# spotify-research/llark

Hardware: AMD Instinct MI355X
Metric: clips/sec (25 s audio + 128-tok prompt) end-to-end fwd (higher is better)
Workload: dtype fp16x2-split(fp32-class) prior + bf16x2-split(fp32-class) llm; 1 GPU; configs[1]+llm: 8x25s clips -> Jukebox VQ-VAE+36-layer prior -> 240x4800 -> projector -> Llama-2-7B fwd (S=371) logits; clips_per_gpu=8, global_batch=8, audio_samples=1048576, seq_len=371, prior_depth=36, prior_precision=f16x2, prior_layernorm_folded=True, parallelism=dp1 (clip-sharded, no collective), debug_overrides=False

## Files before the change

llark_amd/csrc/llama.hip:

```cpp
#include <stdlib.h>

#include "common.h"

namespace llark {

template <typename T>
__global__ void embed_gather_kernel(const long long* __restrict__ ids, const T* __restrict__ table,
                                    float* __restrict__ out, int rows, int width, int vocab, int ldo) {
    const int row = blockIdx.x;
    long long id = ids[row];
    id = id < 0 ? 0 : (id >= vocab ? vocab - 1 : id);
    const T* src = table + (size_t)id * width;
    float* dst = out + (size_t)row * ldo;
    for (int c = threadIdx.x; c < width; c += blockDim.x) dst[c] = (float)src[c];
}

template <int NV>
__global__ __launch_bounds__(256) void rmsnorm_kernel(const float* __restrict__ x, int ldx, int rows, int width,
                                                      const float* __restrict__ w, float eps,
                                                      bf16_t* __restrict__ hi, bf16_t* __restrict__ lo, int ldo) {
    const int lane = threadIdx.x & 63;
    const int row = blockIdx.x * 4 + (threadIdx.x >> 6);
    if (row >= rows) return;
    const int w4 = width >> 2;
    const float4* xr = (const float4*)(x + (size_t)row * ldx);
    const float4* w4p = (const float4*)w;
    float4 v[NV], gw[NV];
#pragma unroll
    for (int k = 0; k < NV; ++k) {
        const int c = lane + 64 * k;
        if (c < w4) {
            v[k] = xr[c];
            gw[k] = w4p[c];
        } else {
            v[k] = gw[k] = make_float4(0.f, 0.f, 0.f, 0.f);
        }
    }
    float s = 0.0f;
#pragma unroll
    for (int k = 0; k < NV; ++k)
        if (lane + 64 * k < w4) s += (v[k].x * v[k].x + v[k].y * v[k].y) + (v[k].z * v[k].z + v[k].w * v[k].w);
    const float var = wave_sum(s) / (float)width;
    const float rstd = 1.0f / sqrtf(var + eps);
    bf16x4_t* hr = (bf16x4_t*)(hi + (size_t)row * ldo);
    bf16x4_t* lr = lo ? (bf16x4_t*)(lo + (size_t)row * ldo) : nullptr;
#pragma unroll
    for (int k = 0; k < NV; ++k) {
        const int c = lane + 64 * k;
        if (c < w4) {
            const float4 g = gw[k];
            float y[4] = {g.x * (v[k].x * rstd), g.y * (v[k].y * rstd), g.z * (v[k].z * rstd), g.w * (v[k].w * rstd)};
            bf16x4_t h, l;
#pragma unroll
            for (int e = 0; e < 4; ++e) {
                h[e] = (bf16_t)y[e];
                l[e] = (bf16_t)(y[e] - (float)h[e]);
            }
            hr[c] = h;
            if (lr) lr[c] = l;
        }
    }
}

__device__ __forceinline__ void store_split(bf16_t* __restrict__ hi, bf16_t* __restrict__ lo, size_t idx, float v) {
    const bf16_t h = (bf16_t)v;
    hi[idx] = h;
    if (lo) lo[idx] = (bf16_t)(v - (float)h);
}

__global__ __launch_bounds__(256) void rope_split_kernel(const float* __restrict__ qkv, int S, int nh, int pos0,
                                                         const float* __restrict__ cos_t, const float* __restrict__ sin_t,
                                                         bf16_t* __restrict__ q, bf16_t* __restrict__ kc,
                                                         bf16_t* __restrict__ vtc, bf16_t* __restrict__ q_lo,
                                                         bf16_t* __restrict__ kc_lo, bf16_t* __restrict__ vtc_lo, int smax,
                                                         const int* __restrict__ pos_dev) {
    __shared__ float sv[64][129];
    if (pos_dev) pos0 = *pos_dev;
    const int hd = 128, H = nh * hd;
    const int s0 = blockIdx.x * 64, h = blockIdx.y, b = blockIdx.z;
    const int ns = (S - s0) < 64 ? (S - s0) : 64;
    for (int i = threadIdx.x; i < ns * 64; i += 256) {
        const int t = i >> 6, d = i & 63;
        const int s = s0 + t, pos = pos0 + s;
        const float* row = qkv + ((size_t)b * S + s) * 3 * H + h * hd;
        const float c = cos_t[(size_t)pos * 64 + d], sn = sin_t[(size_t)pos * 64 + d];
        const float q1 = row[d], q2 = row[d + 64], k1 = row[H + d], k2 = row[H + d + 64];
        const float qa = __fadd_rn(__fmul_rn(q1, c), __fmul_rn(-q2, sn));
        const float qb = __fadd_rn(__fmul_rn(q2, c), __fmul_rn(q1, sn));
        const float ka = __fadd_rn(__fmul_rn(k1, c), __fmul_rn(-k2, sn));
        const float kb = __fadd_rn(__fmul_rn(k2, c), __fmul_rn(k1, sn));
        const size_t qo = (((size_t)b * nh + h) * S + s) * hd;
        const size_t ko = (((size_t)b * nh + h) * smax + pos) * hd;
        store_split(q, q_lo, qo + d, qa);
        store_split(q, q_lo, qo + d + 64, qb);
        store_split(kc, kc_lo, ko + d, ka);
        store_split(kc, kc_lo, ko + d + 64, kb);
    }
    for (int i = threadIdx.x; i < ns * hd; i += 256) {
        const int t = i >> 7, d = i & 127;
        sv[t][d] = qkv[((size_t)b * S + s0 + t) * 3 * H + 2 * H + h * hd + d];
    }
    __syncthreads();
    for (int i = threadIdx.x; i < hd * 64; i += 256) {
        const int d = i >> 6, t = i & 63;
        if (t < ns) store_split(vtc, vtc_lo, (((size_t)b * nh + h) * hd + d) * smax + pos0 + s0 + t, sv[t][d]);
    }
}

__device__ __forceinline__ int k_swz(int key) { return ((key & 3) << 1) | (key & 8); }
__device__ __forceinline__ int k_off(int key, int chunk) { return key * 256 + ((chunk ^ k_swz(key)) << 4); }
__device__ __forceinline__ int v_off(int d, int chunk) { return d * 128 + ((chunk ^ ((d >> 1) & 7)) << 4); }
__device__ __forceinline__ int sub_row(int sub, int i) { return ((sub >> 1) << 5) + ((i >> 2) << 3) + ((sub & 1) << 2) + (i & 3); }

#ifndef ATTN_PREFILL_SM2
#define ATTN_PREFILL_SM2 1
#endif
#ifndef ATTN_PREFILL_PF
#define ATTN_PREFILL_PF 3
#endif
template <bool SPLIT, int NQ, bool P2, bool ALIBI, bool VARLEN = false>
__global__ __launch_bounds__(256) __attribute__((amdgpu_waves_per_eu((NQ == 1 && !SPLIT) ? 3 : 2, (NQ == 1 && !SPLIT) ? 3 : 2))) void attn_prefill_kernel(const bf16_t* __restrict__ q, const bf16_t* __restrict__ kc,
                                                           const bf16_t* __restrict__ vtc, const bf16_t* __restrict__ q_lo,
                                                           const bf16_t* __restrict__ kc_lo, const bf16_t* __restrict__ vtc_lo,
                                                           bf16_t* __restrict__ out, bf16_t* __restrict__ out_lo,
                                                           int S_arg, int nh, int nbh, int past, int smax, float scale,
                                                           const float* __restrict__ alibi_arg, float* __restrict__ lse, int paired,
                                                           const AttnSeqs<VARLEN> vl) {
    extern __shared__ __attribute__((aligned(16))) char smem[];
    const float* alibi = ALIBI ? alibi_arg : nullptr;
    char* sKl = smem + 32768;
    char* sVl = smem + 49152;
    constexpr int BQ = 64 * NQ;
    constexpr float LOG2E = 1.4426950408889634f;
    const int lane = threadIdx.x & 63;
    const int wv = __builtin_amdgcn_readfirstlane(threadIdx.x >> 6);
    const int g = lane >> 4, c = lane & 15;
    const int nt_grid = (S_arg + BQ - 1) / BQ;
    const int np = paired ? (nt_grid + 1) >> 1 : nt_grid;
    int pidx, bhid;
    {
        const int L = blockIdx.x;
        if ((nbh & 7) == 0) {
            bhid = (L & 7) + 8 * (L / (8 * np));
            pidx = (L >> 3) % np;
        } else {
            bhid = L / np;
            pidx = L - bhid * np;
        }
    }
    const int b = bhid / nh, h = bhid - b * nh;
    int S = S_arg, nt = nt_grid;
    size_t qrow0 = (size_t)bhid * S_arg;
    size_t krow0 = (size_t)bhid * smax;
    size_t vcol0 = (size_t)bhid * 128 * smax;
    size_t orow0 = (size_t)b * S_arg;
    if constexpr (VARLEN) {
        int off, len;
        if (!attn_seq_of(vl, b, S_arg, off, len)) return;
        S = len;
        nt = (S + BQ - 1) / BQ;
        if (pidx >= (paired ? (nt + 1) >> 1 : nt)) return;
        qrow0 = (size_t)h * vl.s_total + off;
        krow0 = (size_t)h * smax + off;
        vcol0 = (size_t)h * 128 * smax + off;
        orow0 = (size_t)off;
    }
    const int total = past + S;
    const float slope2 = alibi ? alibi[h] * LOG2E : 0.0f;
    const float scale2 = scale * LOG2E;
    const bf16_t* qb = q + qrow0 * 128;
    const bf16_t* kb = kc + krow0 * 128;
    const bf16_t* vb = vtc + vcol0;
    const bf16_t* kbl = SPLIT ? kc_lo + krow0 * 128 : nullptr;
    const bf16_t* vbl = SPLIT ? vtc_lo + vcol0 : nullptr;

    constexpr int NST = SPLIT ? 1 : 2;
    constexpr int STAGE_BYTES = 32768;
    auto stage_regs = [&](const bf16_t* kbase, const bf16_t* vbase, char* dK, char* dV, int key0) __attribute__((always_inline)) {
        int tid_ = threadIdx.x;
        if constexpr (!SPLIT) asm volatile("" : "+v"(tid_));
#pragma unroll
        for (int i = 0; i < 4; ++i) {
            const int idx = tid_ + i * 256;
            {
                const int key = idx >> 4, ch = idx & 15;
                uint4 val = make_uint4(0, 0, 0, 0);
                if (key0 + key < total) val = *(const uint4*)(kbase + (size_t)(key0 + key) * 128 + ch * 8);
                *(uint4*)(dK + k_off(key, ch)) = val;
            }
            {
                const int d = idx >> 3, ch = idx & 7;
                uint4 val = make_uint4(0, 0, 0, 0);
                const int kk = key0 + ch * 8;
                if (kk + 7 < total) {
                    val = *(const uint4*)(vbase + (size_t)d * smax + kk);
                } else if (kk < total) {
                    const bf16_t* src = vbase + (size_t)d * smax + kk;
                    unsigned short tmp[8];
#pragma unroll
                    for (int e = 0; e < 8; ++e) tmp[e] = (kk + e < total) ? ((const unsigned short*)src)[e] : (unsigned short)0;
                    val = *(uint4*)tmp;
                }
                *(uint4*)(dV + v_off(d, ch)) = val;
            }
        }
    };
    unsigned dko[4], dvo[4];
#pragma unroll
    for (int i = 0; i < 4; ++i) {
        const int j = wv * 4 + i;
        const int krow = 4 * j + (lane >> 4);
        dko[i] = (unsigned)(krow * 128 + (((lane & 15) ^ k_swz(krow)) << 3)) * 2u;
        const int d = 8 * j + (lane >> 3);
        dvo[i] = (unsigned)(d * smax + (((lane & 7) ^ ((d >> 1) & 7)) << 3)) * 2u;
    }
    auto stage_dma = [&](char* dK, char* dV, int key0) __attribute__((always_inline)) {
        const char* kt_base = (const char*)(kb + (size_t)key0 * 128);
        const char* vt_base = (const char*)(vb + key0);
#pragma unroll
        for (int i = 0; i < 4; ++i) {
            const int j = wv * 4 + i;
            __builtin_amdgcn_global_load_lds((const __attribute__((address_space(1))) void*)(kt_base + dko[i]),
                                             (__attribute__((address_space(3))) void*)(dK + j * 1024), 16, 0, 0);
            __builtin_amdgcn_global_load_lds((const __attribute__((address_space(1))) void*)(vt_base + dvo[i]),
                                             (__attribute__((address_space(3))) void*)(dV + j * 1024), 16, 0, 0);
        }
    };
    auto stage = [&](int kt) __attribute__((always_inline)) {
        const int key0 = kt * 64;
        char* base = smem + (NST == 2 ? (kt & 1) * STAGE_BYTES : 0);
        if (!SPLIT && key0 + 64 <= total) {
            stage_dma(base, base + 16384, key0);
        } else {
            stage_regs(kb, vb, base, base + 16384, key0);
            if (SPLIT) {
                __builtin_amdgcn_sched_barrier(0);
                stage_regs(kbl, vbl, sKl, sVl, key0);
            }
        }
    };
    int kaddr[4], vaddr[2];
    {
        const int krow0 = 8 * (c >> 2) + (c & 3);
#pragma unroll
        for (int ks = 0; ks < 4; ++ks) kaddr[ks] = k_off(krow0, ks * 4 + g);
#pragma unroll
        for (int p = 0; p < 2; ++p) vaddr[p] = v_off(c, p * 4 + g);
    }
    auto ksub = [](int sub) { return (32 * (sub >> 1) + 4 * (sub & 1)) * 256; };
#pragma nounroll
    for (int pass = 0; pass < 2; ++pass) {
        const int tile = pass == 0 ? nt - 1 - pidx : pidx;
        if (pass == 1 && (!paired || tile == nt - 1 - pidx)) break;
        if (pass == 1) __syncthreads();
        const int q0 = tile * BQ;
        const int wq0 = q0 + wv * 16 * NQ;
        bf16x8_t qf[NQ][4], ql[SPLIT ? NQ : 1][4];
#pragma unroll
        for (int u = 0; u < NQ; ++u) {
            int qr = wq0 + u * 16 + c;
            qr = qr < S ? qr : S - 1;
#pragma unroll
            for (int ks = 0; ks < 4; ++ks) {
                qf[u][ks] = *(const bf16x8_t*)(qb + (size_t)qr * 128 + ks * 32 + g * 8);
                if (SPLIT) ql[u][ks] = *(const bf16x8_t*)(q_lo + qrow0 * 128 + (size_t)qr * 128 + ks * 32 + g * 8);
            }
        }
        f32x4_t o[NQ][8];
        float m_run[NQ], l_run[NQ];
#pragma unroll
        for (int u = 0; u < NQ; ++u) {
#pragma unroll
            for (int dt = 0; dt < 8; ++dt) o[u][dt] = f32x4_t{0.f, 0.f, 0.f, 0.f};
            m_run[u] = -INFINITY;
            l_run[u] = 0.0f;
        }

        int last_key = past + q0 + BQ - 1;
        if (last_key > total - 1) last_key = total - 1;
        const int ntiles = last_key / 64 + 1;

        if (NST == 2) stage(0);
        for (int kt = 0; kt < ntiles; ++kt) {
            const int key0 = kt * 64;
            if (NST == 2) {
                asm volatile("s_waitcnt vmcnt(0)" ::: "memory");
                __syncthreads();
                if (kt + 1 < ntiles) stage(kt + 1);
            } else {
                __syncthreads();
                stage(kt);
                __syncthreads();
            }
            const char* sK = smem + (NST == 2 ? (kt & 1) * STAGE_BYTES : 0);
            const char* sV = sK + 16384;
            if (key0 > past + wq0 + 16 * NQ - 1) continue;
            f32x4_t st[NQ][4];
            constexpr bool PF = !SPLIT && !ALIBI && (ATTN_PREFILL_PF & 1), PFV = !SPLIT && !ALIBI && NQ == 2 && (ATTN_PREFILL_PF & 2);
            bf16x8_t vfa[PFV ? 8 : 1];
            if constexpr (PF) {
                bf16x8_t kfa[2][4];
#pragma unroll
                for (int sub = 0; sub < 4; ++sub) {
                    kfa[0][sub] = *(const bf16x8_t*)(sK + kaddr[0] + ksub(sub));
#pragma unroll
                    for (int u = 0; u < NQ; ++u) st[u][sub] = f32x4_t{0.f, 0.f, 0.f, 0.f};
                }
#pragma unroll
                for (int ks = 0; ks < 4; ++ks) {
                    __builtin_amdgcn_sched_barrier(0);
                    if (ks < 3) {
#pragma unroll
                        for (int sub = 0; sub < 4; ++sub) kfa[(ks + 1) & 1][sub] = *(const bf16x8_t*)(sK + kaddr[ks + 1] + ksub(sub));
                    }
                    __builtin_amdgcn_sched_barrier(0);
#pragma unroll
                    for (int sub = 0; sub < 4; ++sub)
#pragma unroll
                        for (int u = 0; u < NQ; ++u) st[u][sub] = __builtin_amdgcn_mfma_f32_16x16x32_bf16(kfa[ks & 1][sub], qf[u][ks], st[u][sub], 0, 0, 0);
                }
            } else {
#pragma unroll
            for (int sub = 0; sub < 4; ++sub) {
#pragma unroll
                for (int u = 0; u < NQ; ++u) st[u][sub] = f32x4_t{0.f, 0.f, 0.f, 0.f};
#pragma unroll
                for (int ks = 0; ks < 4; ++ks) {
                    const bf16x8_t kf = *(const bf16x8_t*)(sK + kaddr[ks] + ksub(sub));
                    bf16x8_t kfl;
                    if (SPLIT) kfl = *(const bf16x8_t*)(sKl + kaddr[ks] + ksub(sub));
#pragma unroll
                    for (int u = 0; u < NQ; ++u) {
                        st[u][sub] = __builtin_amdgcn_mfma_f32_16x16x32_bf16(kf, qf[u][ks], st[u][sub], 0, 0, 0);
                        if (SPLIT) {
                            st[u][sub] = __builtin_amdgcn_mfma_f32_16x16x32_bf16(kfl, qf[u][ks], st[u][sub], 0, 0, 0);
                            st[u][sub] = __builtin_amdgcn_mfma_f32_16x16x32_bf16(kf, ql[u][ks], st[u][sub], 0, 0, 0);
                        }
                    }
                }
            }
            }
            if constexpr (PFV) {
                __builtin_amdgcn_sched_barrier(0);
#pragma unroll
                for (int dt = 0; dt < 8; ++dt) vfa[dt] = *(const bf16x8_t*)(sV + vaddr[0] + dt * 2048);
                __builtin_amdgcn_sched_barrier(0);
            }
            const bool need_mask = key0 + 63 > past + wq0 || key0 + 63 >= total;
            bf16x8_t ph[NQ][2], pl[P2 ? NQ : 1][2];
            constexpr bool SM2 = !SPLIT && !P2 && !ALIBI && ATTN_PREFILL_SM2;
            if constexpr (SM2) {
#pragma unroll
                for (int u = 0; u < NQ; ++u) {
                    const int lim = past + wq0 + u * 16 + c;
                    if (need_mask) {
#pragma unroll
                        for (int sub = 0; sub < 4; ++sub)
#pragma unroll
                            for (int r = 0; r < 4; ++r) {
                                const int key = key0 + sub_row(sub, 4 * g + r);
                                if (key > lim || key >= total) st[u][sub][r] = -INFINITY;
                            }
                    }
                    float mloc = fmaxf(fmaxf(st[u][0][0], st[u][0][1]), fmaxf(st[u][0][2], st[u][0][3]));
#pragma unroll
                    for (int sub = 1; sub < 4; ++sub) mloc = fmaxf(fmaxf(fmaxf(st[u][sub][0], st[u][sub][1]), fmaxf(st[u][sub][2], st[u][sub][3])), mloc);
                    {
                        const unsigned xm = __builtin_bit_cast(unsigned, mloc);
                        const auto a = __builtin_amdgcn_permlane16_swap(xm, xm, false, false);
                        const unsigned a0 = a[0], a1 = a[1];
                        mloc = fmaxf(__builtin_bit_cast(float, a0), __builtin_bit_cast(float, a1));
                        const unsigned ym = __builtin_bit_cast(unsigned, mloc);
                        const auto b2 = __builtin_amdgcn_permlane32_swap(ym, ym, false, false);
                        const unsigned b0 = b2[0], b1 = b2[1];
                        mloc = fmaxf(__builtin_bit_cast(float, b0), __builtin_bit_cast(float, b1));
                    }
                    const float mn = fmaxf(m_run[u], mloc * scale2);
                    const bool dead = mn == -INFINITY;
                    const float alpha = dead ? 1.0f : __builtin_amdgcn_exp2f(m_run[u] - mn);
                    const float nmn = dead ? 0.0f : -mn;
                    float rs = 0.0f;
#pragma unroll
                    for (int sub = 0; sub < 4; ++sub)
#pragma unroll
                        for (int r = 0; r < 4; ++r) {
                            const float pv = __builtin_amdgcn_exp2f(__builtin_fmaf(st[u][sub][r], scale2, nmn));
                            rs += pv;
                            ph[u][sub >> 1][(sub & 1) * 4 + r] = (bf16_t)pv;
                        }
                l_run[u] = l_run[u] * alpha + rs;
                    m_run[u] = mn;
                    if (__builtin_amdgcn_ballot_w64(alpha != 1.0f) != 0) {
#pragma unroll
                        for (int dt = 0; dt < 8; ++dt)
#pragma unroll
                            for (int r = 0; r < 4; ++r) o[u][dt][r] *= alpha;
                    }
                }
            } else
#pragma unroll
            for (int u = 0; u < NQ; ++u) {
                const int lim = past + wq0 + u * 16 + c;
                float mloc = -INFINITY;
                if (need_mask || alibi) {
#pragma unroll
                    for (int sub = 0; sub < 4; ++sub)
#pragma unroll
                        for (int r = 0; r < 4; ++r) {
                            const int key = key0 + sub_row(sub, 4 * g + r);
                            float sv = st[u][sub][r] * scale2;
                            if (alibi) sv += slope2 * (float)(key - (total - 1));
                            if (key > lim || key >= total) sv = -INFINITY;
                            st[u][sub][r] = sv;
                            mloc = fmaxf(mloc, sv);
                        }
                } else {
#pragma unroll
                    for (int sub = 0; sub < 4; ++sub)
#pragma unroll
                        for (int r = 0; r < 4; ++r) {
                            st[u][sub][r] *= scale2;
                            mloc = fmaxf(mloc, st[u][sub][r]);
                        }
                }
                mloc = fmaxf(mloc, __shfl_xor(mloc, 16, 64));
                mloc = fmaxf(mloc, __shfl_xor(mloc, 32, 64));
                const float mn = fmaxf(m_run[u], mloc);
                const bool dead = mn == -INFINITY;
                const float alpha = dead ? 1.0f : __builtin_amdgcn_exp2f(m_run[u] - mn);
                float rs = 0.0f;
#pragma unroll
                for (int sub = 0; sub < 4; ++sub)
#pragma unroll
                    for (int r = 0; r < 4; ++r) {
                        const float pv = dead ? 0.0f : __builtin_amdgcn_exp2f(st[u][sub][r] - mn);
                        rs += pv;
                        const bf16_t pb = (bf16_t)pv;
                        ph[u][sub >> 1][(sub & 1) * 4 + r] = pb;
                        if (P2) pl[u][sub >> 1][(sub & 1) * 4 + r] = (bf16_t)(pv - (float)pb);
                    }
                rs += __shfl_xor(rs, 16, 64);
                rs += __shfl_xor(rs, 32, 64);
                l_run[u] = l_run[u] * alpha + rs;
                m_run[u] = mn;
                if (__builtin_amdgcn_ballot_w64(alpha != 1.0f) != 0) {
#pragma unroll
                    for (int dt = 0; dt < 8; ++dt)
#pragma unroll
                        for (int r = 0; r < 4; ++r) o[u][dt][r] *= alpha;
                }
            }
            bf16x8_t vfb[PFV ? 8 : 1];
            if constexpr (PFV) {
                __builtin_amdgcn_sched_barrier(0);
#pragma unroll
                for (int dt = 0; dt < 8; ++dt) vfb[dt] = *(const bf16x8_t*)(sV + vaddr[1] + dt * 2048);
            }
#pragma unroll
            for (int p = 0; p < 2; ++p) {
#pragma unroll
                for (int dt = 0; dt < 8; ++dt) {
                    bf16x8_t vf;
                    if constexpr (PFV) vf = p == 0 ? vfa[dt] : vfb[dt];
                    else vf = *(const bf16x8_t*)(sV + vaddr[p] + dt * 2048);
                    bf16x8_t vfl;
                    if (SPLIT) vfl = *(const bf16x8_t*)(sVl + vaddr[p] + dt * 2048);
#pragma unroll
                    for (int u = 0; u < NQ; ++u) {
                        o[u][dt] = __builtin_amdgcn_mfma_f32_16x16x32_bf16(vf, ph[u][p], o[u][dt], 0, 0, 0);
                        if (P2) o[u][dt] = __builtin_amdgcn_mfma_f32_16x16x32_bf16(vf, pl[u][p], o[u][dt], 0, 0, 0);
                        if (SPLIT) o[u][dt] = __builtin_amdgcn_mfma_f32_16x16x32_bf16(vfl, ph[u][p], o[u][dt], 0, 0, 0);
                    }
                }
            }
        }
#pragma unroll
        for (int u = 0; u < NQ; ++u) {
            const int qi = wq0 + u * 16 + c;
            if (!SPLIT && !P2 && !ALIBI && ATTN_PREFILL_SM2) {
                l_run[u] += __shfl_xor(l_run[u], 16, 64);
                l_run[u] += __shfl_xor(l_run[u], 32, 64);
            }
            if (qi >= S) continue;
            const float inv = l_run[u] > 0.0f ? 1.0f / l_run[u] : 0.0f;
            if (lse && g == 0) lse[qrow0 + qi] = (m_run[u] + log2f(l_run[u])) * 0.6931471805599453f;
            const size_t dst = (orow0 + qi) * (size_t)(nh * 128) + h * 128;
#pragma unroll
            for (int dt = 0; dt < 8; ++dt) {
                bf16x4_t hi4, lo4;
#pragma unroll
                for (int r = 0; r < 4; ++r) {
                    const float v = o[u][dt][r] * inv;
                    hi4[r] = (bf16_t)v;
                    lo4[r] = (bf16_t)(v - (float)hi4[r]);
                }
                *(bf16x4_t*)(out + dst + dt * 16 + 4 * g) = hi4;
                if (SPLIT) *(bf16x4_t*)(out_lo + dst + dt * 16 + 4 * g) = lo4;
            }
        }
    }
}

template <bool SPLIT, bool P2>
static void launch_attn_prefill(hipStream_t st, const bf16_t* q, const bf16_t* kc, const bf16_t* vtc, const bf16_t* q_lo,
                                const bf16_t* kc_lo, const bf16_t* vtc_lo, bf16_t* out, bf16_t* out_lo, int batch, int s, int nh,
                                int past, int smax, float scale, const float* alibi, float* lse) {
    const int lds = 65536;
    const int nbh = batch * nh;
    auto pairs_ok = [&](int nt) { const long wgs = (long)((nt + 1) / 2) * nbh; return nt >= 2 && (wgs >= 2048 || wgs == 512 || wgs == 1024); };
    auto go = [&](auto alibi_c) {
        constexpr bool AL = decltype(alibi_c)::value;
        auto run = [&](auto nq_c) {
            constexpr int NQ = decltype(nq_c)::value;
            const int nt = cdiv(s, 64 * NQ), pr = pairs_ok(nt);
            static PerDeviceOnce once;
            if (once.first()) (void)hipFuncSetAttribute((const void*)attn_prefill_kernel<SPLIT, NQ, P2, AL>, hipFuncAttributeMaxDynamicSharedMemorySize, lds);
            attn_prefill_kernel<SPLIT, NQ, P2, AL><<<(pr ? (nt + 1) / 2 : nt) * nbh, 256, lds, st>>>(q, kc, vtc, q_lo, kc_lo, vtc_lo, out, out_lo, s, nh, nbh, past,
                                                                                           smax, scale, alibi, lse, pr, AttnSeqs<false>{});
        };
        if (!SPLIT && (long)cdiv(s, 128) * nbh >= 1024) run(std::integral_constant<int, SPLIT ? 1 : 2>{});
        else run(std::integral_constant<int, 1>{});
    };
    if (alibi) go(std::true_type{});
    else go(std::false_type{});
}

template <int NW, int UBT>
__device__ __forceinline__ void attn_decode_body(const float* sq, float* sp, float* red, const bf16_t* kc, const bf16_t* vtc,
                                                 const bf16_t* kc_lo, const bf16_t* vtc_lo, bf16_t* __restrict__ out,
                                                 bf16_t* __restrict__ out_lo, int nh, int total, int smax, float scale,
                                                 const float* __restrict__ alibi) {
    constexpr int NT = NW * 64;
    constexpr int UB = UBT;
    constexpr int PARTS = NT / 128;
    const int h = blockIdx.x, b = blockIdx.y;
    const size_t bh = (size_t)b * nh + h;
    const int tid = threadIdx.x, lane = tid & 63, wv = tid >> 6;
    __syncthreads();
    const bf16_t* kb = kc + bh * (size_t)smax * 128;
    const bf16_t* kbl = kc_lo ? kc_lo + bh * (size_t)smax * 128 : nullptr;
    const int chunk = lane & 15, sub = lane >> 4;
    float qv[8];
#pragma unroll
    for (int e = 0; e < 8; ++e) qv[e] = sq[chunk * 8 + e];
    float lmax = -INFINITY;
    constexpr int KSTEP = NW * 4;
    for (int jb = wv * 4 + sub; jb < total + KSTEP - 1; jb += KSTEP * UB) {
        bf16x8_t kv[UB], kl[UB];
#pragma unroll
        for (int u = 0; u < UB; ++u) {
            int j = jb + KSTEP * u;
            j = j < total ? j : total - 1;
            kv[u] = *(const bf16x8_t*)(kb + (size_t)j * 128 + chunk * 8);
            if (kbl) kl[u] = *(const bf16x8_t*)(kbl + (size_t)j * 128 + chunk * 8);
        }
#pragma unroll
        for (int u = 0; u < UB; ++u) {
            const int j = jb + KSTEP * u;
            float s = 0.0f;
            if (kbl) {
#pragma unroll
                for (int e = 0; e < 8; ++e) s = fmaf(qv[e], (float)kv[u][e] + (float)kl[u][e], s);
            } else {
#pragma unroll
                for (int e = 0; e < 8; ++e) s = fmaf(qv[e], (float)kv[u][e], s);
            }
            s += __shfl_xor(s, 1, 64);
            s += __shfl_xor(s, 2, 64);
            s += __shfl_xor(s, 4, 64);
            s += __shfl_xor(s, 8, 64);
            s *= scale;
            if (alibi) s += alibi[blockIdx.x] * (float)(j - (total - 1));
            if (j < total) {
                if (chunk == 0) sp[j] = s;
                lmax = fmaxf(lmax, s);
            }
        }
    }
    lmax = wave_max(lmax);
    if (lane == 0) red[wv] = lmax;
    __syncthreads();
    float mx = red[0];
#pragma unroll
    for (int i = 1; i < NW; ++i) mx = fmaxf(mx, red[i]);
    float lsum = 0.0f;
    const int tpad = (total + 7) & ~7;
    for (int j = tid; j < tpad; j += NT) {
        float p = 0.0f;
        if (j < total) {
            p = expf(sp[j] - mx);
            lsum += p;
        }
        sp[j] = p;
    }
    lsum = wave_sum(lsum);
    __syncthreads();
    if (lane == 0) red[NW + wv] = lsum;
    __syncthreads();
    float tot = 0.0f;
#pragma unroll
    for (int i = 0; i < NW; ++i) tot += red[NW + i];
    const float inv = 1.0f / tot;
    const int d = tid / PARTS, part = tid % PARTS;
    const bf16_t* vr = vtc + (bh * 128 + d) * (size_t)smax;
    const bf16_t* vrl = vtc_lo ? vtc_lo + (bh * 128 + d) * (size_t)smax : nullptr;
    float acc = 0.0f;
    for (int cb = part * 8; cb < tpad; cb += 8 * PARTS * UB) {
        bf16x8_t vv[UB], vl[UB];
#pragma unroll
        for (int u = 0; u < UB; ++u) {
            int c8 = cb + 8 * PARTS * u;
            c8 = c8 < tpad ? c8 : tpad - 8;
            vv[u] = *(const bf16x8_t*)(vr + c8);
            if (vrl) vl[u] = *(const bf16x8_t*)(vrl + c8);
        }
#pragma unroll
        for (int u = 0; u < UB; ++u) {
            const int c8 = cb + 8 * PARTS * u;
            if (c8 < tpad) {
                if (vrl && c8 + 8 > total) {
#pragma unroll
                    for (int e = 0; e < 8; ++e)
                        if (c8 + e < total) acc = fmaf(sp[c8 + e], (float)vv[u][e] + (float)vl[u][e], acc);
                } else if (vrl) {
#pragma unroll
                    for (int e = 0; e < 8; ++e) acc = fmaf(sp[c8 + e], (float)vv[u][e] + (float)vl[u][e], acc);
                } else {
#pragma unroll
                    for (int e = 0; e < 8; ++e) acc = fmaf(sp[c8 + e], (float)vv[u][e], acc);
                }
            }
        }
    }
#pragma unroll
    for (int o = 1; o < PARTS; o <<= 1) acc += __shfl_xor(acc, o, 64);
    if (part == 0) store_split(out, out_lo, (size_t)b * (nh * 128) + h * 128 + d, acc * inv);
}

template <int NW, int UBT, bool ROWS = false>
__global__ __launch_bounds__(NW * 64, (NW >= 16 && UBT == 4) ? 7 : 1) void attn_decode_kernel(const bf16_t* __restrict__ q, bf16_t* kc, bf16_t* vtc,
                                                              const bf16_t* __restrict__ q_lo, bf16_t* kc_lo, bf16_t* vtc_lo,
                                                              bf16_t* __restrict__ out, bf16_t* __restrict__ out_lo,
                                                              int nh, int total, int smax, float scale,
                                                              const int* __restrict__ pos_dev, const float* __restrict__ alibi,
                                                              const float* __restrict__ qkv, const float* __restrict__ cos_t,
                                                              const float* __restrict__ sin_t, unsigned* chain_done) {
    extern __shared__ __attribute__((aligned(16))) char smem[];
    if constexpr (ROWS) {
        const int p = pos_dev[blockIdx.y];
        if (p < 0 || p >= smax) {
            if (threadIdx.x < 128)
                store_split(out, out_lo, (size_t)blockIdx.y * (nh * 128) + blockIdx.x * 128 + threadIdx.x, 0.0f);
            return;
        }
        total = p + 1;
    } else if (pos_dev) total = *pos_dev + 1;
    float* sp = (float*)smem;
    __shared__ float sq[128];
    __shared__ float red[2 * NW];
    const int h = blockIdx.x, b = blockIdx.y;
    const size_t bh = (size_t)b * nh + h;
    const int tid = threadIdx.x, lane = tid & 63, wv = tid >> 6;
    if (qkv) {
        const int pos = total - 1, H = nh * 128;
        const float* row = qkv + (size_t)b * 3 * H + h * 128;
        const bool split = kc_lo != nullptr;
        if (tid < 64) {
            const int d = tid;
            const float c = cos_t[(size_t)pos * 64 + d], sn = sin_t[(size_t)pos * 64 + d];
            const float q1 = row[d], q2 = row[d + 64], k1 = row[H + d], k2 = row[H + d + 64];
            const float qa = __fadd_rn(__fmul_rn(q1, c), __fmul_rn(-q2, sn));
            const float qb = __fadd_rn(__fmul_rn(q2, c), __fmul_rn(q1, sn));
            const float ka = __fadd_rn(__fmul_rn(k1, c), __fmul_rn(-k2, sn));
            const float kb2 = __fadd_rn(__fmul_rn(k2, c), __fmul_rn(k1, sn));
            const bf16_t ha = (bf16_t)qa, hb = (bf16_t)qb;
            sq[d] = (float)ha + (split ? (float)(bf16_t)(qa - (float)ha) : 0.0f);
            sq[d + 64] = (float)hb + (split ? (float)(bf16_t)(qb - (float)hb) : 0.0f);
            const size_t ko = (bh * (size_t)smax + pos) * 128;
            store_split(kc, kc_lo, ko + d, ka);
            store_split(kc, kc_lo, ko + d + 64, kb2);
        } else if (tid >= 128 && tid < 256) {
            const int d = tid - 128;
            store_split(vtc, vtc_lo, (bh * 128 + d) * (size_t)smax + pos, row[2 * H + d]);
        }
    } else if (tid < 128) {
        sq[tid] = (float)q[bh * 128 + tid] + (q_lo ? (float)q_lo[bh * 128 + tid] : 0.0f);
    }
    attn_decode_body<NW, UBT>(sq, sp, red, kc, vtc, kc_lo, vtc_lo, out, out_lo, nh, total, smax, scale, alibi);
    chain_signal(ChainSync{nullptr, 0u, chain_done});
}

__device__ __forceinline__ float clamp_keep_nan(float v, float lim) {
    return (lim > 0.0f && v == v) ? fminf(fmaxf(v, -lim), lim) : v;
}

template <int NW, int UBT>
__global__ __launch_bounds__(NW * 64, (NW >= 16 && UBT == 4) ? 7 : 1) void mpt_attn_decode_kernel(
    const float* __restrict__ qkv, int ldq, int nh, const int* __restrict__ pos_rows, float clip, const float* __restrict__ q_ln_w,
    const float* __restrict__ q_ln_b, const float* __restrict__ k_ln_w, const float* __restrict__ k_ln_b, float eps, bf16_t* kc, bf16_t* vtc,
    bf16_t* kc_lo, bf16_t* vtc_lo, int smax, bf16_t* __restrict__ out, bf16_t* __restrict__ out_lo, float scale,
    const float* __restrict__ alibi) {
    extern __shared__ __attribute__((aligned(16))) char smem[];
    const int pos = pos_rows[blockIdx.y];
    if (pos < 0 || pos >= smax) {
        if (threadIdx.x < 128) store_split(out, out_lo, (size_t)blockIdx.y * (nh * 128) + blockIdx.x * 128 + threadIdx.x, 0.0f);
        return;
    }
    float* sp = (float*)smem;
    __shared__ float sq[128];
    __shared__ float red[2 * NW];
    __shared__ float stat[4];
    const int h = blockIdx.x, b = blockIdx.y, H = nh * 128;
    const size_t bh = (size_t)b * nh + h;
    const int tid = threadIdx.x, lane = tid & 63, wv = tid >> 6;
    const float* row = qkv + (size_t)b * ldq;
    const bool ln = q_ln_w != nullptr, split = kc_lo != nullptr;
    const int d = tid & 127, isk = tid >> 7;
    float x = 0.0f, g = 1.0f, be = 0.0f;
    if (tid < 256) {
        x = clamp_keep_nan(row[isk * H + h * 128 + d], clip);
        if (ln) {
            g = (isk ? k_ln_w : q_ln_w)[h * 128 + d];
            const float* bp = isk ? k_ln_b : q_ln_b;
            be = bp ? bp[h * 128 + d] : 0.0f;
        }
    }
    if (tid >= 128 && tid < 256)
        store_split(vtc, vtc_lo, (bh * 128 + d) * (size_t)smax + pos, clamp_keep_nan(row[2 * H + h * 128 + d], clip));
    if (ln) {
        if (wv < 2) {
            const float4* xr = (const float4*)(row + wv * H);
            const int w4 = H >> 2;
            float s = 0.0f;
            for (int c = lane; c < w4; c += 64) {
                float4 v = xr[c];
                v.x = clamp_keep_nan(v.x, clip), v.y = clamp_keep_nan(v.y, clip), v.z = clamp_keep_nan(v.z, clip), v.w = clamp_keep_nan(v.w, clip);
                s += (v.x + v.y) + (v.z + v.w);
            }
            const float mean = wave_sum(s) / (float)H;
            float q = 0.0f;
            for (int c = lane; c < w4; c += 64) {
                float4 v = xr[c];
                v.x = clamp_keep_nan(v.x, clip), v.y = clamp_keep_nan(v.y, clip), v.z = clamp_keep_nan(v.z, clip), v.w = clamp_keep_nan(v.w, clip);
                const float a = v.x - mean, bb = v.y - mean, cc = v.z - mean, dd = v.w - mean;
                q += (a * a + bb * bb) + (cc * cc + dd * dd);
            }
            const float rstd = 1.0f / sqrtf(wave_sum(q) / (float)H + eps);
            if (lane == 0) stat[2 * wv] = mean, stat[2 * wv + 1] = rstd;
        }
        __syncthreads();
        if (tid < 256) x = (x - stat[2 * isk]) * stat[2 * isk + 1] * g + be;
    }
    if (tid < 128) {
        const bf16_t hi = (bf16_t)x;
        sq[d] = (float)hi + (split ? (float)(bf16_t)(x - (float)hi) : 0.0f);
    } else if (tid < 256) {
        store_split(kc, kc_lo, (bh * (size_t)smax + pos) * 128 + d, x);
    }
    attn_decode_body<NW, UBT>(sq, sp, red, kc, vtc, kc_lo, vtc_lo, out, out_lo, nh, pos + 1, smax, scale, alibi);
}

enum AttnDecodePos { POS_HOST, POS_DEV, POS_ROWS };
struct AttnDecodeArgs {
    const char* name;
    bool fused;
    const void *q, *q_lo;
    const float *qkv, *cos_t, *sin_t, *alibi;
    void *k_cache, *vt_cache, *k_cache_lo, *vt_cache_lo, *out, *out_lo;
    int batch, nh, hd, smax, max_pos;
    AttnDecodePos from;
    long total;
    const int *pos_dev, *pos_rows;
    unsigned* chain_done;
    llark_stream_t stream;
};

static int attn_decode(const AttnDecodeArgs& a) {
    LLARK_REQUIRE(a.k_cache && a.vt_cache && a.out && (a.fused ? a.qkv && a.cos_t && a.sin_t : a.q != nullptr) &&
                      (a.from == POS_HOST || (a.from == POS_DEV ? a.pos_dev : a.pos_rows)), "%s: null pointer", a.name);
    LLARK_REQUIRE(a.hd == 128, "%s: head_dim must be 128 (Llama-2), got %d", a.name, a.hd);
    LLARK_REQUIRE(!a.fused || ((a.k_cache_lo == nullptr) == (a.vt_cache_lo == nullptr) && (a.k_cache_lo == nullptr) == (a.out_lo == nullptr)),
                  "%s: give all lo planes (fp32-class mode) or none", a.name);
    bool ok = a.batch > 0 && a.nh > 0 && a.smax % 8 == 0;
    if (a.from == POS_HOST) ok = ok && a.total > 0 && a.total <= a.smax && (!a.fused || a.total <= a.max_pos);
    if (a.from == POS_DEV) ok = ok && (a.fused || a.smax > 0);
    if (a.from == POS_ROWS) ok = ok && a.smax > 0 && a.smax <= a.max_pos;
    LLARK_REQUIRE(ok, "%s: bad shape batch=%d nh=%d pos=%ld smax=%d max_pos=%d", a.name, a.batch, a.nh, a.total - 1, a.smax, a.max_pos);
    const size_t lds = (a.from == POS_HOST ? (size_t)((a.total + 7) & ~7L) : (size_t)a.smax) * sizeof(float);
    LLARK_REQUIRE(lds <= 128 * 1024, "%s: context too long for the LDS score buffer (total=%ld smax=%d)", a.name, a.total, a.smax);
    const float scale = (float)(1.0 / sqrt((double)a.hd));
    const int total = a.from == POS_HOST ? (int)a.total : 1;
    auto go = [&](auto rows_c) {
        constexpr bool ROWS = decltype(rows_c)::value;
        auto launch = [&](auto kern, int threads) {
            kern<<<dim3(a.nh, a.batch), threads, lds, (hipStream_t)a.stream>>>(
                (const bf16_t*)a.q, (bf16_t*)a.k_cache, (bf16_t*)a.vt_cache, (const bf16_t*)a.q_lo, (bf16_t*)a.k_cache_lo, (bf16_t*)a.vt_cache_lo,
                (bf16_t*)a.out, (bf16_t*)a.out_lo, a.nh, total, a.smax, scale, ROWS ? a.pos_rows : a.pos_dev, a.alibi, a.qkv, a.cos_t, a.sin_t, a.chain_done);
        };
        static PerDeviceOnce once;
        const bool first = once.first();
        if (lds > 48 * 1024 && (first || (int)lds > once.slot())) {
            (void)hipFuncSetAttribute((const void*)attn_decode_kernel<4, 8, ROWS>, hipFuncAttributeMaxDynamicSharedMemorySize, (int)lds);
            (void)hipFuncSetAttribute((const void*)attn_decode_kernel<16, 4, ROWS>, hipFuncAttributeMaxDynamicSharedMemorySize, (int)lds);
            once.slot() = (int)lds;
        }
        if ((long)a.nh * a.batch < 256) launch(attn_decode_kernel<16, 4, ROWS>, 1024);
        else launch(attn_decode_kernel<4, 8, ROWS>, 256);
    };
    if (a.from == POS_ROWS) go(std::true_type{});
    else go(std::false_type{});
    return check_launch(a.name);
}

__global__ __launch_bounds__(256) void ce_rows_kernel(const float* __restrict__ logits, int ldl, int S, int vocab,
                                                      const long long* __restrict__ labels, long long ignore_index,
                                                      float* __restrict__ row_loss) {
    __shared__ float red[8];
    const int s = blockIdx.x, b = blockIdx.y;
    const int row = b * S + s;
    const int lane = threadIdx.x & 63, wv = threadIdx.x >> 6;
    long long tgt = (s + 1 < S) ? labels[(size_t)b * S + s + 1] : ignore_index;
    if (tgt == ignore_index || tgt < 0 || tgt >= vocab) {
        if (threadIdx.x == 0) row_loss[row] = CE_ROW_NOT_COUNTED;
        return;
// ... 375 lines not shown
```

Baseline: 13.54 clips/s.

## Use async LDS DMA with split K/V staging in split-precision prefill attention

```diff
diff --git a/llark_amd/csrc/llama.hip b/llark_amd/csrc/llama.hip
--- a/llark_amd/csrc/llama.hip
+++ b/llark_amd/csrc/llama.hip
@@ -1,4 +1,5 @@
 #include <stdlib.h>
+#include <string.h>
 
 #include "common.h"
 
@@ -118,7 +119,7 @@
 #ifndef ATTN_PREFILL_PF
 #define ATTN_PREFILL_PF 3
 #endif
-template <bool SPLIT, int NQ, bool P2, bool ALIBI, bool VARLEN = false>
+template <bool SPLIT, int NQ, bool P2, bool ALIBI, bool VARLEN = false, bool RSTG = false>
 __global__ __launch_bounds__(256) __attribute__((amdgpu_waves_per_eu((NQ == 1 && !SPLIT) ? 3 : 2, (NQ == 1 && !SPLIT) ? 3 : 2))) void attn_prefill_kernel(const bf16_t* __restrict__ q, const bf16_t* __restrict__ kc,
                                                            const bf16_t* __restrict__ vtc, const bf16_t* __restrict__ q_lo,
                                                            const bf16_t* __restrict__ kc_lo, const bf16_t* __restrict__ vtc_lo,
@@ -175,20 +176,21 @@
     const bf16_t* vbl = SPLIT ? vtc_lo + vcol0 : nullptr;
 
     constexpr int NST = SPLIT ? 1 : 2;
+    constexpr bool SDMA = SPLIT && !RSTG;
     constexpr int STAGE_BYTES = 32768;
-    auto stage_regs = [&](const bf16_t* kbase, const bf16_t* vbase, char* dK, char* dV, int key0) __attribute__((always_inline)) {
+    auto stage_regs = [&](const bf16_t* kbase, const bf16_t* vbase, char* dK, char* dV, int key0, auto do_k, auto do_v) __attribute__((always_inline)) {
         int tid_ = threadIdx.x;
         if constexpr (!SPLIT) asm volatile("" : "+v"(tid_));
 #pragma unroll
         for (int i = 0; i < 4; ++i) {
             const int idx = tid_ + i * 256;
-            {
+            if constexpr (decltype(do_k)::value) {
                 const int key = idx >> 4, ch = idx & 15;
                 uint4 val = make_uint4(0, 0, 0, 0);
                 if (key0 + key < total) val = *(const uint4*)(kbase + (size_t)(key0 + key) * 128 + ch * 8);
                 *(uint4*)(dK + k_off(key, ch)) = val;
             }
-            {
+            if constexpr (decltype(do_v)::value) {
                 const int d = idx >> 3, ch = idx & 7;
                 uint4 val = make_uint4(0, 0, 0, 0);
                 const int kk = key0 + ch * 8;
@@ -232,12 +234,55 @@
         if (!SPLIT && key0 + 64 <= total) {
             stage_dma(base, base + 16384, key0);
         } else {
-            stage_regs(kb, vb, base, base + 16384, key0);
+            stage_regs(kb, vb, base, base + 16384, key0, std::true_type{}, std::true_type{});
             if (SPLIT) {
                 __builtin_amdgcn_sched_barrier(0);
-                stage_regs(kbl, vbl, sKl, sVl, key0);
-            }
-        }
+                stage_regs(kbl, vbl, sKl, sVl, key0, std::true_type{}, std::true_type{});
+            }
+        }
+    };
+    auto stage_k = [&](int kt) __attribute__((always_inline)) {
+        const int key0 = kt * 64;
+        if (key0 + 64 <= total) {
+            const char* kh = (const char*)(kb + (size_t)key0 * 128);
+            const char* kl = (const char*)(kbl + (size_t)key0 * 128);
+#pragma unroll
+            for (int i = 0; i < 4; ++i) {
+                const int j = wv * 4 + i;
+                __builtin_amdgcn_global_load_lds((const __attribute__((address_space(1))) void*)(kh + dko[i]),
+                                                 (__attribute__((address_space(3))) void*)(smem + j * 1024), 16, 0, 0);
+                __builtin_amdgcn_global_load_lds((const __attribute__((address_space(1))) void*)(kl + dko[i]),
+                                                 (__attribute__((address_space(3))) void*)(sKl + j * 1024), 16, 0, 0);
+            }
+        } else {
+            stage_regs(kb, vb, smem, smem + 16384, key0, std::true_type{}, std::false_type{});
+            __builtin_amdgcn_sched_barrier(0);
+            stage_regs(kbl, vbl, sKl, sVl, key0, std::true_type{}, std::false_type{});
+        }
+    };
+    auto stage_v = [&](int kt) __attribute__((always_inline)) {
+        const int key0 = kt * 64;
+        if (key0 + 64 <= total) {
+            const char* vh = (const char*)(vb + key0);
+            const char* vl = (const char*)(vbl + key0);
+#pragma unroll
+            for (int i = 0; i < 4; ++i) {
+                const int j = wv * 4 + i;
+                __builtin_amdgcn_global_load_lds((const __attribute__((address_space(1))) void*)(vh + dvo[i]),
+                                                 (__attribute__((address_space(3))) void*)(smem + 16384 + j * 1024), 16, 0, 0);
+                __builtin_amdgcn_global_load_lds((const __attribute__((address_space(1))) void*)(vl + dvo[i]),
+                                                 (__attribute__((address_space(3))) void*)(sVl + j * 1024), 16, 0, 0);
+            }
+        } else {
+            stage_regs(kb, vb, smem, smem + 16384, key0, std::false_type{}, std::true_type{});
+            __builtin_amdgcn_sched_barrier(0);
+            stage_regs(kbl, vbl, sKl, sVl, key0, std::false_type{}, std::true_type{});
+        }
+    };
+    auto mid_tile = [&](int kt, int ntiles) __attribute__((always_inline)) {
+        asm volatile("s_waitcnt vmcnt(0)" ::: "memory");
+        __syncthreads();
+        if (kt + 1 < ntiles) stage_k(kt + 1);
     };
     int kaddr[4], vaddr[2];
     {
@@ -255,6 +300,7 @@
         if (pass == 1) __syncthreads();
         const int q0 = tile * BQ;
         const int wq0 = q0 + wv * 16 * NQ;
+        if constexpr (SDMA) stage_k(0);
         bf16x8_t qf[NQ][4], ql[SPLIT ? NQ : 1][4];
 #pragma unroll
         for (int u = 0; u < NQ; ++u) {
@@ -283,7 +329,11 @@
         if (NST == 2) stage(0);
         for (int kt = 0; kt < ntiles; ++kt) {
             const int key0 = kt * 64;
-            if (NST == 2) {
+            if constexpr (SDMA) {
+                asm volatile("s_waitcnt vmcnt(0)" ::: "memory");
+                __syncthreads();
+                stage_v(kt);
+            } else if (NST == 2) {
                 asm volatile("s_waitcnt vmcnt(0)" ::: "memory");
                 __syncthreads();
                 if (kt + 1 < ntiles) stage(kt + 1);
@@ -294,7 +344,10 @@
             }
             const char* sK = smem + (NST == 2 ? (kt & 1) * STAGE_BYTES : 0);
             const char* sV = sK + 16384;
-            if (key0 > past + wq0 + 16 * NQ - 1) continue;
+            if (key0 > past + wq0 + 16 * NQ - 1) {
+                if constexpr (SDMA) mid_tile(kt, ntiles);
+                continue;
+            }
             f32x4_t st[NQ][4];
             constexpr bool PF = !SPLIT && !ALIBI && (ATTN_PREFILL_PF & 1), PFV = !SPLIT && !ALIBI && NQ == 2 && (ATTN_PREFILL_PF & 2);
             bf16x8_t vfa[PFV ? 8 : 1];
@@ -450,6 +503,7 @@
                         for (int r = 0; r < 4; ++r) o[u][dt][r] *= alpha;
                 }
             }
+            if constexpr (SDMA) mid_tile(kt, ntiles);
             bf16x8_t vfb[PFV ? 8 : 1];
             if constexpr (PFV) {
                 __builtin_amdgcn_sched_barrier(0);
@@ -499,6 +553,11 @@
             }
         }
     }
+}
+
+static bool attn_split_staging_regs() {
+    const char* e = getenv("LLARK_ATTN_SPLIT_STAGING");
+    return e && strcmp(e, "regs") == 0;
 }
 
 template <bool SPLIT, bool P2>
@@ -510,16 +569,18 @@
     auto pairs_ok = [&](int nt) { const long wgs = (long)((nt + 1) / 2) * nbh; return nt >= 2 && (wgs >= 2048 || wgs == 512 || wgs == 1024); };
     auto go = [&](auto alibi_c) {
         constexpr bool AL = decltype(alibi_c)::value;
-        auto run = [&](auto nq_c) {
+        auto run = [&](auto nq_c, auto rstg_c) {
             constexpr int NQ = decltype(nq_c)::value;
+            constexpr bool RS = decltype(rstg_c)::value;
             const int nt = cdiv(s, 64 * NQ), pr = pairs_ok(nt);
             static PerDeviceOnce once;
-            if (once.first()) (void)hipFuncSetAttribute((const void*)attn_prefill_kernel<SPLIT, NQ, P2, AL>, hipFuncAttributeMaxDynamicSharedMemorySize, lds);
-            attn_prefill_kernel<SPLIT, NQ, P2, AL><<<(pr ? (nt + 1) / 2 : nt) * nbh, 256, lds, st>>>(q, kc, vtc, q_lo, kc_lo, vtc_lo, out, out_lo, s, nh, nbh, past,
+            if (once.first()) (void)hipFuncSetAttribute((const void*)attn_prefill_kernel<SPLIT, NQ, P2, AL, false, RS>, hipFuncAttributeMaxDynamicSharedMemorySize, lds);
+            attn_prefill_kernel<SPLIT, NQ, P2, AL, false, RS><<<(pr ? (nt + 1) / 2 : nt) * nbh, 256, lds, st>>>(q, kc, vtc, q_lo, kc_lo, vtc_lo, out, out_lo, s, nh, nbh, past,
                                                                                            smax, scale, alibi, lse, pr, AttnSeqs<false>{});
         };
-        if (!SPLIT && (long)cdiv(s, 128) * nbh >= 1024) run(std::integral_constant<int, SPLIT ? 1 : 2>{});
-        else run(std::integral_constant<int, 1>{});
+        if (!SPLIT && (long)cdiv(s, 128) * nbh >= 1024) run(std::integral_constant<int, SPLIT ? 1 : 2>{}, std::false_type{});
+        else if (SPLIT && attn_split_staging_regs()) run(std::integral_constant<int, 1>{}, std::integral_constant<bool, SPLIT>{});
+        else run(std::integral_constant<int, 1>{}, std::false_type{});
     };
     if (alibi) go(std::true_type{});
     else go(std::false_type{});
```

Measured after the change: 13.60 clips/s, median of 5. Within noise of the previous version (+0.4%).

## Use 32-key tiles in split-precision attention prefill to halve LDS and raise occupancy

Applied to the files above, without the earlier changes.

```diff
diff --git a/llark_amd/csrc/llama.hip b/llark_amd/csrc/llama.hip
--- a/llark_amd/csrc/llama.hip
+++ b/llark_amd/csrc/llama.hip
@@ -109,7 +109,10 @@
 
 __device__ __forceinline__ int k_swz(int key) { return ((key & 3) << 1) | (key & 8); }
 __device__ __forceinline__ int k_off(int key, int chunk) { return key * 256 + ((chunk ^ k_swz(key)) << 4); }
-__device__ __forceinline__ int v_off(int d, int chunk) { return d * 128 + ((chunk ^ ((d >> 1) & 7)) << 4); }
+template <int KT>
+__device__ __forceinline__ int v_swz(int d) { return (d >> 1) & (KT / 8 - 1); }
+template <int KT>
+__device__ __forceinline__ int v_off(int d, int chunk) { return d * (2 * KT) + ((chunk ^ v_swz<KT>(d)) << 4); }
 __device__ __forceinline__ int sub_row(int sub, int i) { return ((sub >> 1) << 5) + ((i >> 2) << 3) + ((sub & 1) << 2) + (i & 3); }
 
 #ifndef ATTN_PREFILL_SM2
@@ -118,8 +121,15 @@
 #ifndef ATTN_PREFILL_PF
 #define ATTN_PREFILL_PF 3
 #endif
-template <bool SPLIT, int NQ, bool P2, bool ALIBI, bool VARLEN = false>
-__global__ __launch_bounds__(256) __attribute__((amdgpu_waves_per_eu((NQ == 1 && !SPLIT) ? 3 : 2, (NQ == 1 && !SPLIT) ? 3 : 2))) void attn_prefill_kernel(const bf16_t* __restrict__ q, const bf16_t* __restrict__ kc,
+#ifndef ATTN_PREFILL_KT_SPLIT
+#define ATTN_PREFILL_KT_SPLIT 32
+#endif
+#ifndef ATTN_PREFILL_WAVES_SPLIT
+#define ATTN_PREFILL_WAVES_SPLIT 4
+#endif
+constexpr int attn_prefill_waves(bool split, int nq, int kt) { return split ? (kt == 32 ? ATTN_PREFILL_WAVES_SPLIT : 2) : (nq == 1 ? 3 : 2); }
+template <bool SPLIT, int NQ, bool P2, bool ALIBI, bool VARLEN = false, int KT = 64>
+__global__ __launch_bounds__(256) __attribute__((amdgpu_waves_per_eu(attn_prefill_waves(SPLIT, NQ, KT), attn_prefill_waves(SPLIT, NQ, KT)))) void attn_prefill_kernel(const bf16_t* __restrict__ q, const bf16_t* __restrict__ kc,
                                                            const bf16_t* __restrict__ vtc, const bf16_t* __restrict__ q_lo,
                                                            const bf16_t* __restrict__ kc_lo, const bf16_t* __restrict__ vtc_lo,
                                                            bf16_t* __restrict__ out, bf16_t* __restrict__ out_lo,
@@ -128,8 +138,10 @@
                                                            const AttnSeqs<VARLEN> vl) {
     extern __shared__ __attribute__((aligned(16))) char smem[];
     const float* alibi = ALIBI ? alibi_arg : nullptr;
-    char* sKl = smem + 32768;
-    char* sVl = smem + 49152;
+    static_assert(KT == 64 || (KT == 32 && SPLIT), "the LDS-DMA image and the fragment prefetch of the plain kernels are laid out for 64 keys");
+    constexpr int PLANE = KT * 256, NSUB = KT / 16, NP = KT / 32;
+    char* sKl = smem + 2 * PLANE;
+    char* sVl = smem + 3 * PLANE;
     constexpr int BQ = 64 * NQ;
     constexpr float LOG2E = 1.4426950408889634f;
     const int lane = threadIdx.x & 63;
@@ -175,12 +187,12 @@
     const bf16_t* vbl = SPLIT ? vtc_lo + vcol0 : nullptr;
 
     constexpr int NST = SPLIT ? 1 : 2;
-    constexpr int STAGE_BYTES = 32768;
+    constexpr int STAGE_BYTES = 2 * PLANE;
     auto stage_regs = [&](const bf16_t* kbase, const bf16_t* vbase, char* dK, char* dV, int key0) __attribute__((always_inline)) {
         int tid_ = threadIdx.x;
-        if constexpr (!SPLIT) asm volatile("" : "+v"(tid_));
-#pragma unroll
-        for (int i = 0; i < 4; ++i) {
+        if constexpr (!SPLIT || KT == 32) asm volatile("" : "+v"(tid_));
+#pragma unroll
+        for (int i = 0; i < KT / 16; ++i) {
             const int idx = tid_ + i * 256;
             {
                 const int key = idx >> 4, ch = idx & 15;
@@ -189,7 +201,7 @@
                 *(uint4*)(dK + k_off(key, ch)) = val;
             }
             {
-                const int d = idx >> 3, ch = idx & 7;
+                const int d = idx >> (KT == 64 ? 3 : 2), ch = idx & (KT / 8 - 1);
                 uint4 val = make_uint4(0, 0, 0, 0);
                 const int kk = key0 + ch * 8;
                 if (kk + 7 < total) {
@@ -201,7 +213,7 @@
                     for (int e = 0; e < 8; ++e) tmp[e] = (kk + e < total) ? ((const unsigned short*)src)[e] : (unsigned short)0;
                     val = *(uint4*)tmp;
                 }
-                *(uint4*)(dV + v_off(d, ch)) = val;
+                *(uint4*)(dV + v_off<KT>(d, ch)) = val;
             }
         }
     };
@@ -227,25 +239,25 @@
         }
     };
     auto stage = [&](int kt) __attribute__((always_inline)) {
-        const int key0 = kt * 64;
+        const int key0 = kt * KT;
         char* base = smem + (NST == 2 ? (kt & 1) * STAGE_BYTES : 0);
-        if (!SPLIT && key0 + 64 <= total) {
-            stage_dma(base, base + 16384, key0);
+        if (!SPLIT && key0 + KT <= total) {
+            stage_dma(base, base + PLANE, key0);
         } else {
-            stage_regs(kb, vb, base, base + 16384, key0);
+            stage_regs(kb, vb, base, base + PLANE, key0);
             if (SPLIT) {
                 __builtin_amdgcn_sched_barrier(0);
                 stage_regs(kbl, vbl, sKl, sVl, key0);
             }
         }
     };
-    int kaddr[4], vaddr[2];
+    int kaddr[4], vaddr[NP];
     {
         const int krow0 = 8 * (c >> 2) + (c & 3);
 #pragma unroll
         for (int ks = 0; ks < 4; ++ks) kaddr[ks] = k_off(krow0, ks * 4 + g);
 #pragma unroll
-        for (int p = 0; p < 2; ++p) vaddr[p] = v_off(c, p * 4 + g);
+        for (int p = 0; p < NP; ++p) vaddr[p] = v_off<KT>(c, p * 4 + g);
     }
     auto ksub = [](int sub) { return (32 * (sub >> 1) + 4 * (sub & 1)) * 256; };
 #pragma nounroll
@@ -278,11 +290,11 @@
 
         int last_key = past + q0 + BQ - 1;
         if (last_key > total - 1) last_key = total - 1;
-        const int ntiles = last_key / 64 + 1;
+        const int ntiles = last_key / KT + 1;
 
         if (NST == 2) stage(0);
         for (int kt = 0; kt < ntiles; ++kt) {
-            const int key0 = kt * 64;
+            const int key0 = kt * KT;
             if (NST == 2) {
                 asm volatile("s_waitcnt vmcnt(0)" ::: "memory");
                 __syncthreads();
@@ -293,9 +305,9 @@
                 __syncthreads();
             }
             const char* sK = smem + (NST == 2 ? (kt & 1) * STAGE_BYTES : 0);
-            const char* sV = sK + 16384;
+            const char* sV = sK + PLANE;
             if (key0 > past + wq0 + 16 * NQ - 1) continue;
-            f32x4_t st[NQ][4];
+            f32x4_t st[NQ][NSUB];
             constexpr bool PF = !SPLIT && !ALIBI && (ATTN_PREFILL_PF & 1), PFV = !SPLIT && !ALIBI && NQ == 2 && (ATTN_PREFILL_PF & 2);
             bf16x8_t vfa[PFV ? 8 : 1];
             if constexpr (PF) {
@@ -321,7 +333,7 @@
                 }
             } else {
 #pragma unroll
-            for (int sub = 0; sub < 4; ++sub) {
+            for (int sub = 0; sub < NSUB; ++sub) {
 #pragma unroll
                 for (int u = 0; u < NQ; ++u) st[u][sub] = f32x4_t{0.f, 0.f, 0.f, 0.f};
 #pragma unroll
@@ -346,8 +358,8 @@
                 for (int dt = 0; dt < 8; ++dt) vfa[dt] = *(const bf16x8_t*)(sV + vaddr[0] + dt * 2048);
                 __builtin_amdgcn_sched_barrier(0);
             }
-            const bool need_mask = key0 + 63 > past + wq0 || key0 + 63 >= total;
-            bf16x8_t ph[NQ][2], pl[P2 ? NQ : 1][2];
+            const bool need_mask = key0 + KT - 1 > past + wq0 || key0 + KT - 1 >= total;
+            bf16x8_t ph[NQ][NP], pl[P2 ? NQ : 1][NP];
             constexpr bool SM2 = !SPLIT && !P2 && !ALIBI && ATTN_PREFILL_SM2;
             if constexpr (SM2) {
 #pragma unroll
@@ -404,7 +416,7 @@
                 float mloc = -INFINITY;
                 if (need_mask || alibi) {
 #pragma unroll
-                    for (int sub = 0; sub < 4; ++sub)
+                    for (int sub = 0; sub < NSUB; ++sub)
 #pragma unroll
                         for (int r = 0; r < 4; ++r) {
                             const int key = key0 + sub_row(sub, 4 * g + r);
@@ -416,7 +428,7 @@
                         }
                 } else {
 #pragma unroll
-                    for (int sub = 0; sub < 4; ++sub)
+                    for (int sub = 0; sub < NSUB; ++sub)
 #pragma unroll
                         for (int r = 0; r < 4; ++r) {
                             st[u][sub][r] *= scale2;
@@ -430,7 +442,7 @@
                 const float alpha = dead ? 1.0f : __builtin_amdgcn_exp2f(m_run[u] - mn);
                 float rs = 0.0f;
 #pragma unroll
-                for (int sub = 0; sub < 4; ++sub)
+                for (int sub = 0; sub < NSUB; ++sub)
 #pragma unroll
                     for (int r = 0; r < 4; ++r) {
                         const float pv = dead ? 0.0f : __builtin_amdgcn_exp2f(st[u][sub][r] - mn);
@@ -457,14 +469,14 @@
                 for (int dt = 0; dt < 8; ++dt) vfb[dt] = *(const bf16x8_t*)(sV + vaddr[1] + dt * 2048);
             }
 #pragma unroll
-            for (int p = 0; p < 2; ++p) {
+            for (int p = 0; p < NP; ++p) {
 #pragma unroll
                 for (int dt = 0; dt < 8; ++dt) {
                     bf16x8_t vf;
                     if constexpr (PFV) vf = p == 0 ? vfa[dt] : vfb[dt];
-                    else vf = *(const bf16x8_t*)(sV + vaddr[p] + dt * 2048);
+                    else vf = *(const bf16x8_t*)(sV + vaddr[p] + dt * (32 * KT));
                     bf16x8_t vfl;
-                    if (SPLIT) vfl = *(const bf16x8_t*)(sVl + vaddr[p] + dt * 2048);
+                    if (SPLIT) vfl = *(const bf16x8_t*)(sVl + vaddr[p] + dt * (32 * KT));
 #pragma unroll
                     for (int u = 0; u < NQ; ++u) {
                         o[u][dt] = __builtin_amdgcn_mfma_f32_16x16x32_bf16(vf, ph[u][p], o[u][dt], 0, 0, 0);
@@ -505,17 +517,18 @@
 static void launch_attn_prefill(hipStream_t st, const bf16_t* q, const bf16_t* kc, const bf16_t* vtc, const bf16_t* q_lo,
                                 const bf16_t* kc_lo, const bf16_t* vtc_lo, bf16_t* out, bf16_t* out_lo, int batch, int s, int nh,
                                 int past, int smax, float scale, const float* alibi, float* lse) {
-    const int lds = 65536;
     const int nbh = batch * nh;
     auto pairs_ok = [&](int nt) { const long wgs = (long)((nt + 1) / 2) * nbh; return nt >= 2 && (wgs >= 2048 || wgs == 512 || wgs == 1024); };
     auto go = [&](auto alibi_c) {
         constexpr bool AL = decltype(alibi_c)::value;
+        constexpr int KT = (SPLIT && !AL) ? ATTN_PREFILL_KT_SPLIT : 64;
+        const int lds = 4 * KT * 256;
         auto run = [&](auto nq_c) {
             constexpr int NQ = decltype(nq_c)::value;
             const int nt = cdiv(s, 64 * NQ), pr = pairs_ok(nt);
             static PerDeviceOnce once;
-            if (once.first()) (void)hipFuncSetAttribute((const void*)attn_prefill_kernel<SPLIT, NQ, P2, AL>, hipFuncAttributeMaxDynamicSharedMemorySize, lds);
-            attn_prefill_kernel<SPLIT, NQ, P2, AL><<<(pr ? (nt + 1) / 2 : nt) * nbh, 256, lds, st>>>(q, kc, vtc, q_lo, kc_lo, vtc_lo, out, out_lo, s, nh, nbh, past,
+            if (once.first()) (void)hipFuncSetAttribute((const void*)attn_prefill_kernel<SPLIT, NQ, P2, AL, false, KT>, hipFuncAttributeMaxDynamicSharedMemorySize, lds);
+            attn_prefill_kernel<SPLIT, NQ, P2, AL, false, KT><<<(pr ? (nt + 1) / 2 : nt) * nbh, 256, lds, st>>>(q, kc, vtc, q_lo, kc_lo, vtc_lo, out, out_lo, s, nh, nbh, past,
                                                                                            smax, scale, alibi, lse, pr, AttnSeqs<false>{});
         };
         if (!SPLIT && (long)cdiv(s, 128) * nbh >= 1024) run(std::integral_constant<int, SPLIT ? 1 : 2>{});
```

New measurement: 13.74 clips/s before, 13.75 clips/s after, median of 3. About the same (+0.1%).
